# tatsy/opengl-raytracer

Hardware: AMD Instinct MI355X
Metric: Mrays/s at 1920x1080, 8 bounces (higher is better)
Workload: dtype f32

## Files before the change

opengl-raytracer_amd/csrc/glrtx.hip:

```cpp
#include "glrtx.h"

#include <hip/hip_runtime.h>

#include <algorithm>
#include <cmath>
#include <cstdarg>
#include <cstdio>
#include <cstdlib>
#include <cstring>
#include <new>
#include <limits>
#include <string>
#include <vector>

#include "glrt_host.h"
#include "pt_kernel.hip.h"
#include "lbvh.hip.h"
#include "sahl.hip.h"
#include "refit.hip.h"
#include "query.hip.h"
#include "features.hip.h"
#include "denoise.hip.h"
#include "reproject.hip.h"
#include "../host/reproject_setup.h"
// ... 1079 lines not shown
    if (fed) {
        FeedHost *fh = slot->feed_h;
        for (int i = 0; i < n_frames; i++) fh->seeds[i] = make_float2(seeds_xy[2 * i], seeds_xy[2 * i + 1]);
        __atomic_store_n(&fh->frames_pub, (unsigned)n_frames, __ATOMIC_RELEASE);
        w.feed_host = slot->feed_h_dev;
        w.feed_dev = (FeedDev *)slot->feed_d.p;
        w.feed_plane_f4 = plane_f4;
        w.feed_margin = 64 * 4 * grid;
        if (const char *v = std::getenv("GLRTX_FEED_MARGIN")) w.feed_margin = std::max(0, std::atoi(v));
    } else {
        if (n_frames > 1) {
            if ((rc = ensure(c, c->wfSeeds, (size_t)n_frames * sizeof(float2)))) return rc;
            HIP_TRY(c, hipMemcpyAsync(c->wfSeeds.p, seeds_xy, (size_t)n_frames * sizeof(float2), hipMemcpyHostToDevice, c->stream));
            w.seeds = (const float2 *)c->wfSeeds.p;
            w.seeds_in_lds = n_frames <= kLdsSeeds ? 1 : 0;
        }
        if (n_frames > 1 || slot || adapt) {
            if ((rc = ensure(c, planeBuf, (size_t)std::max(n_planes, 1) * plane_f4 * sizeof(float4)))) return rc;
            w.planes = (float4 *)planeBuf.p;
        }
    }
    w.block_paths = block_paths;
    w.gss_div = (slot && !fed) ? 0 : 4 * grid;
    if (const char *v = std::getenv("GLRTX_GSS_DIV")) w.gss_div = std::max(0, std::atoi(v));
    w.suspend_max = kSuspendMax;
    if (const char *v = std::getenv("GLRTX_SUSPEND_MAX")) w.suspend_max = std::max(0, std::min(64, std::atoi(v)));
    w.trip_limit = (int)std::min<long long>(INT32_MAX, 64ll * std::max(p->n_samples, 1) * (p->max_depth + 2) + 64);
    if (vol) w.trip_limit = (int)std::min<long long>(INT32_MAX, 64ll * std::max(p->n_samples, 1) * 9 * (p->max_depth + 2) + 64);
    if (const char *v = std::getenv("GLRTX_TRIP_LIMIT")) w.trip_limit = std::max(1, std::atoi(v));
    w.err = c->guard_dev;
    {
        const size_t max_id = ids - 1;
        const size_t max_sidx = (size_t)kWfSetPlanes * state_entries + (size_t)grid * block_paths - 1;
        const size_t slice_f4 = 2 * (size_t)2 * 2 * block_paths  + (2 * (size_t)block_paths * sizeof(unsigned) + 15) / 16 ;
        static_assert(kWgSuspendAt + (size_t)kSuspendF4 * kBlockThreads == kWgQueueF4, "the suspend area closes a workgroup's slice");
        bool ok = slice_f4 <= kWgSuspendAt && max_id < (size_t)WF_INVALID && 2 * max_sidx + 1 < (size_t)WF_INVALID && (size_t)grid * block_paths <= state_entries &&
                  (size_t)kWfStatePlanes * state_entries * sizeof(float4) < ((size_t)1 << 32) && (block_paths & (block_paths - 1)) == 0 && block_paths >= 256 &&
                  block_paths <= kWgPathsMax && slice_f4 <= kWgQueueF4 && queueBuf.bytes >= (size_t)grid * kWgQueueF4 * sizeof(float4) &&
                  stateBuf.bytes >= state_bytes && w.ids == state_entries && grid >= 1 && (size_t)grid <= wg_slots &&
                  p->max_depth <= kWfDepthMax && p->n_samples <= kWfSampleMax && workPtr != nullptr;
        if (vol) ok = ok && p->n_samples <= kWfVolSampleMax && c->ext_flags == GLRTX_EXT_VOLUME && c->have_volume && c->vol.density != nullptr &&
                      c->vol.temperature != nullptr && c->n_spheres == 0 && !vine && fetch == 0 && !compact;
        if (!fed && n_frames > 1) ok = ok && c->wfSeeds.bytes >= (size_t)n_frames * sizeof(float2);
        if (w.planes) ok = ok && planeBuf.bytes >= (size_t)std::max(n_planes, 1) * plane_f4 * sizeof(float4);
        if (adapt) ok = ok && !fed && !slot && w.planes && c->ad_selected && c->ad_tiles == (int)(total >> 6) && c->adList.bytes >= (total >> 6) * sizeof(int) &&
                      c->adMask.bytes >= (total >> 6) && c->adHalf.bytes >= (size_t)c->ad_pitch * c->owned_rows && c->ad_pitch == c->pitch_bytes;
        if (fed) ok = ok && n_frames >= 1 && n_frames <= fed_cap && fed_cap <= kFeedMaxFrames && slot->feed_d.bytes >= sizeof(FeedDev) && w.feed_host != nullptr &&
                      slot->chunks[(n_frames - 1) / kFeedChunkFrames].p != nullptr && slot->chunk_bytes == frame_bytes;
        if (!ok) return fail(c, GLRTX_EDEVICE, "internal: wgwf launch shapes inconsistent (ids %zu, max id %zu, grid %d of %zu slots (%d per CU), block_paths %d, frames %d, fed %d)", ids, max_id,
                             grid, wg_slots, per_cu, block_paths, n_frames, (int)fed);
        (void)queue_bytes_max;
    }
    glrtx_ctx::LaunchRec *rec = nullptr;
    if ((rc = next_launch_rec(c, rec))) return rc;
    if (slot && slot->used) HIP_TRY(c, hipStreamWaitEvent(rstream, slot->acc_done, 0));
    if (ctx_state && c->state_used) HIP_TRY(c, hipStreamWaitEvent(rstream, c->state_done, 0));
    HIP_TRY(c, hipMemsetAsync(workPtr, 0, sizeof(unsigned), rstream));
    if (fed) {
        hipLaunchKernelGGL(feed_prefill_kernel, dim3(1), dim3(64), 0, rstream, (FeedDev *)slot->feed_d.p, (const FeedHost *)slot->feed_h_dev, n_frames);
        HIP_TRY(c, hipGetLastError());
    }
    HIP_TRY(c, hipEventRecord(rec->ev0, rstream));
    c->last_kernel = vol ? (adapt ? "pt_render_wgwf (volume, adaptive)" : "pt_render_wgwf (volume)")
                   : adapt ? (vine ? "pt_render_wgwf (adaptive, list scan)" : "pt_render_wgwf (adaptive)") : vine ? "pt_render_wgwf (list scan)" : "pt_render_wgwf";
    c->counters_stale = c->counters_stale || c->count_rays;
    const VolArgs va = vol ? c->vol : VolArgs{};
    hipLaunchKernelGGL(kernel, dim3(grid), dim3(kBlockThreads), lds, rstream, a, w, workPtr, (float4 *)queueBuf.p, adapt ? (const int *)c->adList.p : nullptr,
// ... 2097 lines not shown
```

opengl-raytracer_amd/csrc/pt_kernel.hip.h:

```cpp
#pragma once
#include <hip/hip_runtime.h>
#include <stdint.h>

#include "trav_asm.hip.h"
#include "scan_asm.hip.h"

namespace glrtx {

constexpr int kBlockThreads = 256;
constexpr int kTile = 16;
constexpr int REF_ABSENT = INT32_MIN;
constexpr int REF_FIN = INT32_MIN;
constexpr int kMaxLdsMaterials = 256;
constexpr int kMaxLdsLights = 64;
constexpr int kTopForks = 128;

constexpr float PT_EPS = 1.0e-4f;
constexpr float PT_INFTY = 1.0e8f;
constexpr float PT_PI = 3.14159274101257324f;
constexpr float PT_2PI = 6.28318548202514648f;

struct DevScene {
    const float4 *forks;
    const float4 *nodes0;
// ... 1422 lines not shown
    int total;
    int tiles8_x;
    int refill_min;
    int block_paths;
    int gss_div;
    int suspend_max;
    int trip_limit;
    unsigned *err;
    FeedHost *feed_host;
    FeedDev *feed_dev;
    size_t feed_plane_f4;
    int feed_margin;
    const float2 *seeds;
    int seeds_in_lds;
    float4 *planes;
    int n_frames;
    int tiles_per_frame;
    DEV void split(int id, int &frame, int &pid) const {
        if (n_frames > 1) { frame = (int)((unsigned)id / (unsigned)total); pid = id - frame * total; }
        else { frame = 0; pid = id; }
    }
};
constexpr int kWfStatePlanes = 2 * kWfSetPlanes;
constexpr int kWfDepthMax = 255;
constexpr int kWfSampleMax = (1 << 20) - 1;
constexpr int kWfVolSampleMax = (1 << 16) - 1;
constexpr unsigned kWfVolShift = 24;
constexpr unsigned kWfVolPassed = 9;
constexpr unsigned WF_PENDING = 1u << 28;
constexpr unsigned WF_FINISHING = 1u << 29;
constexpr unsigned WF_RESOLVED = 1u << 30;
constexpr unsigned WF_ACCEPTED = 1u << 31;
constexpr unsigned WF_INVALID = 0xFFFFFFFFu;
constexpr int kSuspendMax = 24;
constexpr float kHitSuspended = -1.0f;
constexpr int kSuspendF4 = 4;
constexpr int kRefillMin = 16;
#ifdef GLRTX_FAULT_INJECT
constexpr unsigned kFaultPoison = 0xFFFFFFFEu;
#endif

DEV bool wf_pixel(const KernelArgs &a, const WfArgs &w, int id, int &lx, int &lrow) {
    int frame, pid;
    w.split(id, frame, pid);
    const int t = pid >> 6, k = pid & 63;
    lx = (t % w.tiles8_x) * 8 + (k & 7);
    lrow = (t / w.tiles8_x) * 8 + (k >> 3);
    return lx < a.width && lrow < a.owned_rows;
}

DEV float2 wf_seed(const KernelArgs &a, const WfArgs &w, const float *cam, int id) {
    if (w.n_frames > 1) {
        int frame, pid;
        w.split(id, frame, pid);
        if (w.seeds_in_lds) {
            const float *sd = cam + kCamFloatsPadded + 2 * frame;
            return make_float2(sd[0], sd[1]);
        }
        if (w.feed_dev != nullptr) {
            const nfloat2 v = ((glb_cf2)&w.feed_dev->seeds[0])[frame];
            return make_float2(v.x, v.y);
        }
        const nfloat2 v = ((glb_cf2)w.seeds)[frame];
        return make_float2(v.x, v.y);
    }
    return make_float2(a.seed_x, a.seed_y);
// ... 5 lines not shown
        w.split(id, frame, pid);
        typedef __attribute__((address_space(1))) nfloat4 *glb_f4;
        const glb_f4 chunk = (glb_f4)w.feed_dev->chunks[frame / kFeedChunkFrames];
        const size_t slot = (size_t)(frame % kFeedChunkFrames) * (size_t)a.n_samples + sample;
        nfloat4 v; v.x = fmin_c(Lx, 100.0f); v.y = fmin_c(Ly, 100.0f); v.z = fmin_c(Lz, 100.0f); v.w = 1.0f;
        __builtin_nontemporal_store(v, &chunk[slot * w.feed_plane_f4 + (size_t)lrow * (size_t)a.pitch_f4 + lx]);
    } else if (w.planes != nullptr) {
        int frame, pid;
        w.split(id, frame, pid);
        const size_t slot = (size_t)frame * (size_t)a.n_samples + sample;
        st_stream(&w.planes[(slot * (size_t)a.owned_rows + (size_t)lrow) * (size_t)a.pitch_f4 + lx],
                  make_float4(fmin_c(Lx, 100.0f), fmin_c(Ly, 100.0f), fmin_c(Lz, 100.0f), 1.0f));
    } else {
        float4 *px = a.accum + (size_t)lrow * a.pitch_f4 + lx;
        float4 acc = *px;
        acc.x = acc.x + fmin_c(Lx, 100.0f);
        acc.y = acc.y + fmin_c(Ly, 100.0f);
        acc.z = acc.z + fmin_c(Lz, 100.0f);
        acc.w = acc.w + 1.0f;
        *px = acc;
    }
}

DEV bool wf_start(const KernelArgs &a, const WfArgs &w, const float *cam, int id, int lx, int lrow, Rng &rng, float fcx, float fcy, Path &P, unsigned &sample) {
    for (;;) {
        if ((int)sample >= a.n_samples) return false;
        camera_ray(a, cam, rng, fcx, fcy, P);
        if (a.max_depth > 0) return true;
        wf_add_sample(a, w, id, lx, lrow, sample, 0.0f, 0.0f, 0.0f);
        sample++;
    }
}

DEV bool wf_generate_one(const KernelArgs &a, const WfArgs &w, const float *cam, int id, unsigned sidx, float4 &ray_o, float4 &ray_d) {
    int lx, lrow;
    bool go = false;
    const float2 sd = wf_seed(a, w, cam, id);
    Rng rng = {0.f, 0.f, sd.x, sd.y};
    Path P;
    unsigned sample = 0;
    if (wf_pixel(a, w, id, lx, lrow)) {
        const int gy = local_row_to_y(a, lrow);
        const float fcx = (float)lx + 0.5f, fcy = (float)gy + 0.5f;
        rng.x = fcx / (float)a.width; rng.y = fcy / (float)a.height;
        go = wf_start(a, w, cam, id, lx, lrow, rng, fcx, fcy, P, sample);
    }
    if (go) {
        st_stream(w.A(0, sidx), make_float4(P.ox, P.oy, P.oz, rng.x));
        st_stream(w.A(1, sidx), make_float4(P.dx, P.dy, P.dz, rng.y));
        st_stream(w.A(2, sidx), make_float4(1.f, 1.f, 1.f, __uint_as_float(sample << 8)));
        st_stream(w.A(3, sidx), make_float4(0.f, 0.f, 0.f, __uint_as_float((unsigned)id)));
        ray_o = make_float4(P.ox, P.oy, P.oz, __uint_as_float(sidx * 2u));
        ray_d = make_float4(P.dx, P.dy, P.dz, 0.f);
    } else st_stream(w.A(3, sidx), make_float4(0.f, 0.f, 0.f, __uint_as_float(WF_INVALID)));
    return go;
}

constexpr int kWfVolEnd = 0, kWfVolNext = 1, kWfVolExit = 2;
DEV const VolArgs *wgwf_vol();
DEV int wf_vol_trial(const KernelArgs &a, const WfArgs &w, unsigned sidx, Rng &rng, Path &P, const Hit &h, unsigned k) {
    if (h.tri < 0) { P.Lx = 1.0f; P.Ly = 0.0f; P.Lz = 1.0f; return kWfVolEnd; }
    const float ox = P.ox, oy = P.oy, oz = P.oz, dx = P.dx, dy = P.dy, dz = P.dz;
    float t = 0.0f;
    bool pass = false;
    for (int i = 0; i < 256; i++) {
        const VolArgs &vo = *wgwf_vol();
        const float dm = vo.density_max;
        t = t - lp_log(fmax_c(1.0f - pt_rand(rng), PT_EPS)) / (dm * VOL_SIGT);
        if (t >= h.t) { pass = true; break; }
        const float density = vol_lookup(vo.density, vo, ox + t * dx, oy + t * dy, oz + t * dz);
        if (density / dm > pt_rand(rng)) { pass = true; break; }
    }
    if (!pass) { P.Lx = 0.0f; P.Ly = 0.0f; P.Lz = 0.0f; return kWfVolEnd; }
    {
        unsigned si = sidx;
        asm volatile("" : "+v"(si));
        const float4 b = ld_stream(w.A(2, si)), l = ld_stream(w.A(3, si));
        P.bx = b.x; P.by = b.y; P.bz = b.z; P.Lx = l.x; P.Ly = l.y; P.Lz = l.z;
    }
    if (t >= h.t) {
        const float te = h.t + PT_EPS;
        P.ox = ox + te * dx; P.oy = oy + te * dy; P.oz = oz + te * dz;
    } else {
        P.ox = ox + t * dx; P.oy = oy + t * dy; P.oz = oz + t * dz;
        float R, G, B;
        const VolArgs &vo = *wgwf_vol();
        vol_blackbody(vol_lookup(vo.temperature, vo, P.ox, P.oy, P.oz), R, G, B);
// ... 140 lines not shown
#define GLRTX_STEPS_PER_TRIP 6
#endif
constexpr int kWgCtlWords = 32;
constexpr int kWgPathsMax = 4096;
constexpr size_t kWgSuspendAt = 8 * (size_t)kWgPathsMax + (size_t)kWgPathsMax / 2;
constexpr size_t kWgQueueF4 = kWgSuspendAt + (size_t)kSuspendF4 * kBlockThreads;
#ifndef GLRTX_PRIO_TRAVERSE
#define GLRTX_PRIO_TRAVERSE 3
#define GLRTX_PRIO_SHADE 0
#endif
#ifndef GLRTX_WGWF_WAVES
#define GLRTX_WGWF_WAVES 4
#endif

#ifdef GLRTX_PHASE_STATS
__device__ unsigned long long g_phase_cycles[8];
__device__ uint4 g_trip_log[16][64];
#define PH_STAMP(var) const unsigned long long var = __builtin_amdgcn_s_memtime()
#define PH_ADD(i, t0, t1) do { if (threadIdx.x == 0) atomicAdd(&g_phase_cycles[i], (t1) - (t0)); } while (0)
#else
#define PH_STAMP(var)
#define PH_ADD(i, t0, t1)
#endif

#ifdef GLRTX_RAY_LOG
struct RayLog { float4 *rays; uint2 *trips; unsigned long long cap_rays; unsigned cap_trips; unsigned on; };
__device__ RayLog g_ray_log;
__device__ unsigned long long g_ray_log_n;
__device__ unsigned g_ray_log_trips;
#endif

DEV int wgwf_suspend_max();

template <bool VINE, int FETCH>
DEV void wg_traverse_phase(const KernelArgs &a, const WfArgs &w, const float4 *root, int *stack, const float4 *rq, int n_rays,
                           unsigned *ray_head, unsigned *light_bits, unsigned long long &rays, float4 *suspend_area) {
    const int lane = threadIdx.x & 63;
    const uint2 *ranks = reinterpret_cast<const uint2 *>(light_bits + kWgPathsMax / 32);
    if (VINE) {
        for (;;) {
            int base = 0;
            if (lane == 0) base = (int)atomicAdd(ray_head, 64u);
            base = __builtin_amdgcn_readfirstlane(base);
            if (base >= n_rays) break;
            float4 o = make_float4(0.f, 0.f, 0.f, __uint_as_float(WF_INVALID)), d = o;
            if (base + lane < n_rays) { o = ld_stream(&rq[2 * (size_t)(base + lane)]); d = ld_stream(&rq[2 * (size_t)(base + lane) + 1]); }
            const unsigned r = __float_as_uint(o.w);
            const bool shadow = (r & 1u) != 0u;
            const Hit h = trav_scan<true>(a.sc, o.x, o.y, o.z, d.x, d.y, d.z, r != WF_INVALID, shadow ? shadow_limit(d.w, a.sc.shadow_limited) : PT_INFTY,
                                          shadow ? d.w : -__builtin_inff());
            if (r != WF_INVALID) {
                rays++;
                if (r & 1u) { if (nee_accepted(d.w, h.t, h.tri >= 0)) atomicOr(&light_bits[r >> 6], 1u << ((r >> 1) & 31u)); }
                else st_stream(w.H(r >> 1), make_float4(h.t, __int_as_float(h.tri), h.u, h.v));
            }
        }
        return;
    }
    const unsigned long long lt_mask = (1ull << lane) - 1ull;
    const float4 none = make_float4(0.f, 0.f, 0.f, __uint_as_float(WF_INVALID));
    float4 cur_o = none, cur_d = none;
    float cur_ix = 0.f, cur_iy = 0.f, cur_iz = 0.f;
    int cur_pos = 0, cur_cnt = 0;
    auto fetch = [&](float4 &o, float4 &d) -> int {
        int base = 0;
        if (lane == 0) base = (int)atomicAdd(ray_head, 64u);
        base = __builtin_amdgcn_readfirstlane(base);
        int cnt = n_rays - base;
        cnt = cnt < 0 ? 0 : (cnt > 64 ? 64 : cnt);
        if (lane < cnt) {
            o = ld_stream(&rq[2 * (size_t)(base + lane)]);
            d = ld_stream(&rq[2 * (size_t)(base + lane) + 1]);
            cur_ix = frcp(d.x); cur_iy = frcp(d.y); cur_iz = frcp(d.z);
            const bool shadow = (__float_as_uint(o.w) & 1u) != 0u;
            float t0;
            if (a.sc.root_boxed && !box_pass(root[0], root[1], o.x, o.y, o.z, cur_ix, cur_iy, cur_iz, shadow ? shadow_limit(d.w, a.sc.shadow_limited) : PT_INFTY, t0))
                d.w = __uint_as_float(__float_as_uint(d.w) | 0x80000000u);
        }
        return cnt;
    };
    cur_cnt = fetch(cur_o, cur_d);
    bool exhausted = cur_cnt == 0;
    const bool fetched_any = cur_cnt > 0;
    bool active = false;
    bool unsaved = false;
    unsigned rid = 0;
    Trav T;
    T.cur = 0; T.sp = 0;
    T.h.t = PT_INFTY; T.h.tri = -1; T.h.u = 0.f; T.h.v = 0.f;
#ifdef GLRTX_STEP_TIMING
    StepTiming step_timing;
#endif
    float4 *const susp = suspend_area + (size_t)kSuspendF4 * threadIdx.x;
    {
        const float4 s3 = susp[3];
        if (s3.z != 0.0f) {
            const float4 s0 = susp[0], s1 = susp[1], s2 = susp[2];
            susp[3] = make_float4(0.f, 0.f, 0.f, 0.f);
            T.ox = s0.x; T.oy = s0.y; T.oz = s0.z;
            rid = __float_as_uint(w.H(__float_as_uint(s0.w) >> 1)->y);
#ifdef GLRTX_FAULT_INJECT
            const bool fault_dropped = rid == kFaultPoison;
#endif
            T.dx = s1.x; T.dy = s1.y; T.dz = s1.z; T.stop_d = s1.w;
            T.ix = frcp(T.dx); T.iy = frcp(T.dy); T.iz = frcp(T.dz);
// ... 105 lines not shown
            bool fin = trav_step<true, CP>(a.sc, stack, T, ranks);
#pragma unroll
            for (int k = 1; k < GLRTX_STEPS_PER_TRIP; k++)
                if (!fin) fin = trav_step<true, CP>(a.sc, stack, T, ranks);
#else
#ifdef GLRTX_STEP_TIMING
            trav_steps_asm<FETCH>(a.sc, stack, T, (unsigned)(uintptr_t)ranks, step_timing);
#else
            trav_steps_asm<FETCH>(a.sc, stack, T, (unsigned)(uintptr_t)ranks);
#endif
            const bool fin = T.cur == REF_FIN;
#endif
            if (fin) {
                active = false;
                unsaved = true;
            }
        }
#ifdef GLRTX_PHASE_STATS
        ph_step += __builtin_amdgcn_s_memtime() - sb0;
#endif
    }
    if (unsaved) save_hit();
#ifdef GLRTX_PHASE_STATS
    if (threadIdx.x == 0) { atomicAdd(&g_phase_cycles[5], ph_refill); atomicAdd(&g_phase_cycles[6], ph_refills); atomicAdd(&g_phase_cycles[7], ph_step); }
#endif
#ifdef GLRTX_STEP_TIMING
    atomicAdd(&g_step_timing[0], (unsigned long long)step_timing.n);
    atomicAdd(&g_step_timing[1], (unsigned long long)step_timing.t);
    atomicAdd(&g_step_timing[2], (unsigned long long)step_timing.w);
#endif
}

template <bool VOL = false>
DEV void wg_shade_phase(const KernelArgs &a, const WfArgs &w, const float4 *lds_mats, const float *cam, const unsigned *light_bits, int n_paths,
                        float4 *rq_next, unsigned *n_rays_next, unsigned *n_paths_next, unsigned cur_base, unsigned next_base, unsigned long long &rays,
                        unsigned *moved) {
    const int lane = threadIdx.x & 63;
    const unsigned long long lt_mask = (1ull << lane) - 1ull;
    for (int j0 = 0; j0 < n_paths; j0 += kBlockThreads) {
        const int i = j0 + (int)threadIdx.x;
        bool push_ext = false, push_sh = false, requeue = false, has4 = false;
        unsigned id = WF_INVALID;
        float4 ro = make_float4(0.f, 0.f, 0.f, 0.f), rd = ro, rsd = ro, st2 = ro, st3 = ro, st4 = ro;
        const bool light_accepted = i < n_paths && ((light_bits[i >> 5] >> (i & 31)) & 1u) != 0u;
        if (i < n_paths)
            wf_shade_path<VOL>(a, w, lds_mats, cam, id, cur_base + (unsigned)i, light_accepted, push_ext, push_sh, requeue, ro, rd, rsd, st2, st3, st4, has4, rays);
        const unsigned long long me = __ballot(push_ext), ms = __ballot(push_sh), mq = __ballot(requeue), mp = me | ms | mq;
        const unsigned long long mv = __ballot(id != WF_INVALID);
        unsigned br = 0, bp = 0;
        if (lane == 0) {
            if (mv & ~mq) *moved = 1u;
            if (mp) {
                br = atomicAdd(n_rays_next, (unsigned)(__popcll(me) + __popcll(ms)));
                bp = atomicAdd(n_paths_next, (unsigned)__popcll(mp));
            }
        }
        br = __builtin_amdgcn_readfirstlane(br);
        bp = __builtin_amdgcn_readfirstlane(bp);
        const unsigned pos_next = bp + (unsigned)__popcll(mp & lt_mask);
        const unsigned sidx_next = next_base + pos_next;
        if (push_ext || push_sh || requeue) {
            st_stream(w.A(0, sidx_next), ro);
            st_stream(w.A(1, sidx_next), rd);
            st_stream(w.A(2, sidx_next), st2);
            st_stream(w.A(3, sidx_next), st3);
            if (has4) st_stream(w.A(4, sidx_next), st4);
        }
#ifdef GLRTX_FAULT_INJECT
        if (requeue) {
            *w.H(cur_base + (unsigned)i) = make_float4(kHitSuspended, __uint_as_float(kFaultPoison), 0.f, 0.f);
            *w.H(sidx_next) = make_float4(kHitSuspended, 0.f, 0.f, 0.f);
        }
#else
        if (requeue) *w.H(cur_base + (unsigned)i) = make_float4(kHitSuspended, __uint_as_float(sidx_next * 2u), 0.f, 0.f);
#endif
        if (push_ext) {
            float4 *r = rq_next + 2 * (size_t)(br + __popcll(me & lt_mask));
            r[0] = make_float4(ro.x, ro.y, ro.z, __uint_as_float(sidx_next * 2u));
            r[1] = make_float4(rd.x, rd.y, rd.z, 0.f);
        }
        if (push_sh) {
            float4 *r = rq_next + 2 * (size_t)(br + __popcll(me) + __popcll(ms & lt_mask));
            r[0] = make_float4(ro.x, ro.y, ro.z, __uint_as_float(pos_next * 2u + 1u));
            r[1] = rsd;
        }
    }
}

struct WgwfKernArgs {
    KernelArgs a;
    WfArgs w;
    unsigned *work_counter;
    float4 *wg_queues;
    const int *adapt_list;
    const unsigned *adapt_count;
    VolArgs vol;
};
DEV const WgwfKernArgs *wgwf_kernargs() {
    auto p = __builtin_amdgcn_kernarg_segment_ptr();
    asm volatile("" : "+s"(p));
    return (const WgwfKernArgs *)p;
}

DEV int wgwf_suspend_max() { return wgwf_kernargs()->w.suspend_max; }
DEV const VolArgs *wgwf_vol() { return &wgwf_kernargs()->vol; }

template <bool VOL = false>
DEV void wg_feed_topup(int kWgPaths, unsigned *ctl, int cur, unsigned *work_counter) {
    const WgwfKernArgs *k = wgwf_kernargs();
    FeedHost *fh = k->w.feed_host;
    FeedDev *fd = k->w.feed_dev;
    int lane = threadIdx.x;
    if constexpr (VOL) asm volatile("" : "+v"(lane));
    const int tpf = k->w.tiles_per_frame, gss_div = k->w.gss_div;
    const int np = (int)ctl[4 + cur];
// ... 90 lines not shown
                                                                                  const int * , const unsigned * , const VolArgs ) {
    constexpr bool ADAPT = (FETCH & kWgwfAdaptive) != 0;
    constexpr bool VOL = (FETCH & kWgwfVolume) != 0;
    constexpr int NODE_FETCH = FETCH & ~(kWgwfAdaptive | kWgwfVolume);
    static_assert(!VOL || (!VINE && NODE_FETCH == 0), "the V form has the one-record-per-lane fetch on DevScene::nodes only");
    extern __shared__ __attribute__((aligned(16))) unsigned char lds_raw[];
    float4 *lds_mats = reinterpret_cast<float4 *>(lds_raw);
    const int mat_f4 = a.sc.lds_head_f4;
    unsigned char *pl = lds_raw + (size_t)mat_f4 * sizeof(float4);
    int *stack = reinterpret_cast<int *>(pl) + 2 * threadIdx.x;
    pl += (size_t)2 * a.sc.stack_entries * kBlockThreads * sizeof(int);
    unsigned *ctl = reinterpret_cast<unsigned *>(pl);
    float4 *lds_root = reinterpret_cast<float4 *>(pl + kWgCtlWords * sizeof(unsigned));
    float *lds_cam = reinterpret_cast<float *>(pl + kWgCtlWords * sizeof(unsigned) + 32);
    unsigned *light_bits = reinterpret_cast<unsigned *>(pl + kWgCtlWords * sizeof(unsigned) + 32 + kCamFloatsPadded * 4 + kLdsSeeds * 8);
    if (threadIdx.x < kCamFloats) lds_cam[threadIdx.x] = a.cam[threadIdx.x];
    if (w.seeds_in_lds && (int)threadIdx.x < 2 * w.n_frames) lds_cam[kCamFloatsPadded + threadIdx.x] = reinterpret_cast<const float *>(w.seeds)[threadIdx.x];
    if (threadIdx.x == 64) lds_root[0] = a.sc.root_lo;
    if (threadIdx.x == 65) lds_root[1] = a.sc.root_hi;
    float4 *rayQ = wg_queues + (size_t)blockIdx.x * kWgQueueF4;
    if (a.sc.mats_in_lds) stage_mats(a, lds_mats);
    stage_lights(a, lds_mats);
    if (FETCH & kWgwfCompact) {
        uint2 *lds_ranks = reinterpret_cast<uint2 *>(light_bits + kWgPathsMax / 32);
        for (int i = threadIdx.x; i < a.sc.n_crank; i += kBlockThreads) lds_ranks[i] = a.sc.cranks[i];
    }

    const int kWgPaths = w.block_paths;
    unsigned long long rays = 0;
#ifdef GLRTX_PHASE_STATS
    if (threadIdx.x == 0 && (blockIdx.x & 63) == 0 && blockIdx.x / 64 < 16)
        g_trip_log[blockIdx.x / 64][0].y = (unsigned)(__builtin_amdgcn_s_memtime() >> 4);
#endif
    if (threadIdx.x == 0) { ctl[2] = 0u; ctl[3] = 0u; ctl[4] = 0u; ctl[5] = 0u; ctl[7] = 0u; ctl[10] = 0u; ctl[11] = 0u; ctl[12] = 0u; ctl[13] = 0u; ctl[14] = 0u; ctl[15] = 0u; ctl[16] = 0u; ctl[17] = 0u; ctl[18] = 0u; }
    if (!VINE) rayQ[kWgSuspendAt + (size_t)kSuspendF4 * threadIdx.x + 3] = make_float4(0.f, 0.f, 0.f, 0.f);
    int cur = 0;
    __syncthreads();
    for (;;) {
        PH_STAMP(pg0);
        unsigned tid_topup = threadIdx.x;
        asm volatile("" : "+v"(tid_topup));
        if (wgwf_kernargs()->w.feed_dev != nullptr) {
            if (tid_topup < 64u) wg_feed_topup<VOL>(kWgPaths, ctl, cur, work_counter);
        } else if (tid_topup == 0u) {
            const int n_tiles = (ADAPT ? (int)*wgwf_kernargs()->adapt_count : wgwf_kernargs()->w.tiles_per_frame) * wgwf_kernargs()->w.n_frames;
            int want = (kWgPaths - (int)ctl[4 + cur]) >> 6;
            int base = 0, got = 0;
            const int gss_div = wgwf_kernargs()->w.gss_div;
            if (want > 0 && ctl[7] == 0u && gss_div > 0) {
                const int left = n_tiles - (int)__hip_atomic_load(work_counter, __ATOMIC_RELAXED, __HIP_MEMORY_SCOPE_AGENT);
                const int share = left > 0 ? (left + gss_div - 1) / gss_div : 1;
                want = want < share ? want : share;
            }
            if (want > 0 && ctl[7] == 0u && ctl[13] == 0u) {
                base = (int)atomicAdd(work_counter, (unsigned)want);
                got = base < n_tiles ? (want < n_tiles - base ? want : n_tiles - base) : 0;
                if (base + want >= n_tiles) ctl[7] = 1u;
            }
            ctl[0] = (unsigned)base; ctl[6] = (unsigned)got; ctl[14] = 0u;
            ctl[12] = got > 0 ? 0u : ctl[12] + 1u;
        }
        __syncthreads();
        if (ctl[13] != 0u) break;
        const bool look_again = ctl[14] != 0u;
        {
            const int got = (int)ctl[6] * 64, tile0 = (int)ctl[0];
            {
                unsigned tid = threadIdx.x;
                asm volatile("" : "+v"(tid));
                if (tid < kWgPathsMax / 32) light_bits[tid] = 0u;
            }
            const int nr = (int)ctl[2 + cur], np = (int)ctl[4 + cur];
            float4 *rq_w = rayQ + 2 * ((size_t)cur * 2 * kWgPaths + nr);
            const WgwfKernArgs *kt = wgwf_kernargs();
            const unsigned new_base = kt->w.set_base(cur, (int)blockIdx.x) + (unsigned)np;
            for (int k = threadIdx.x; k < got; k += kBlockThreads) {
                int id = tile0 * 64 + k;
                if (ADAPT) {
                    const int g = tile0 + (k >> 6), n_active = (int)*kt->adapt_count;
                    const int frame = g / n_active;
                    id = frame * kt->w.total + kt->adapt_list[g - frame * n_active] * 64 + (k & 63);
                }
                float4 ro = make_float4(0.f, 0.f, 0.f, __uint_as_float(WF_INVALID)), rd = ro;
                const bool go = wf_generate_one(kt->a, kt->w, lds_cam, id, new_base + (unsigned)k, ro, rd);
                rq_w[2 * k] = ro;
                rq_w[2 * k + 1] = rd;
                (void)go;
            }
            __syncthreads();
            if (tid_topup == 0u) { ctl[2 + cur] = (unsigned)(nr + got); ctl[4 + cur] = (unsigned)(np + got); ctl[1] = 0u; }
        }
        __syncthreads();
        PH_STAMP(pg1);
        PH_ADD(0, pg0, pg1);
        const int n_rays = (int)ctl[2 + cur], n_paths = (int)ctl[4 + cur];
        if (n_paths == 0) {
            if (look_again) continue;
            break;
        }
        const float4 *rq = rayQ + 2 * ((size_t)cur * 2 * kWgPaths);

#ifdef GLRTX_RAY_LOG
        if (g_ray_log.on) {
            if (threadIdx.x == 0) {
                const unsigned long long base = atomicAdd(&g_ray_log_n, (unsigned long long)n_rays);
                ctl[9] = 0u;
                if (base + (unsigned long long)n_rays <= g_ray_log.cap_rays) {
                    const unsigned t = atomicAdd(&g_ray_log_trips, 1u);
                    if (t < g_ray_log.cap_trips) { g_ray_log.trips[t] = make_uint2((unsigned)base, (unsigned)n_rays); ctl[8] = (unsigned)base; ctl[9] = 1u; }
                }
            }
            __syncthreads();
            if (ctl[9]) {
                float4 *dst = g_ray_log.rays + 2 * (size_t)ctl[8];
                for (int i = threadIdx.x; i < 2 * n_rays; i += kBlockThreads) dst[i] = rq[i];
            }
            __syncthreads();
        }
#endif
        PH_STAMP(pt0);
        __builtin_amdgcn_s_setprio(GLRTX_PRIO_TRAVERSE);
        wg_traverse_phase<VINE, NODE_FETCH>(a, w, lds_root, stack, rq, n_rays, &ctl[1], light_bits, rays, rayQ + kWgSuspendAt);
        __builtin_amdgcn_s_setprio(GLRTX_PRIO_SHADE);
        PH_STAMP(pt1);
        __syncthreads();
        PH_STAMP(pt2);
        PH_ADD(1, pt0, pt1);
        PH_ADD(2, pt1, pt2);

        const WgwfKernArgs *ks = wgwf_kernargs();
        wg_shade_phase<VOL>(ks->a, ks->w, lds_mats, lds_cam, light_bits, n_paths, rayQ + 2 * ((size_t)(cur ^ 1) * 2 * kWgPaths),
                            &ctl[2 + (cur ^ 1)], &ctl[4 + (cur ^ 1)], ks->w.set_base(cur, (int)blockIdx.x), ks->w.set_base(cur ^ 1, (int)blockIdx.x), rays, &ctl[10]);
        PH_STAMP(ps1);
        __syncthreads();
        PH_STAMP(ps2);
        PH_ADD(3, pt2, ps1);
        PH_ADD(4, ps1, ps2);
#ifdef GLRTX_PHASE_STATS
        if (threadIdx.x == 0 && (blockIdx.x & 63) == 0 && blockIdx.x / 64 < 16) {
            uint4 *lg = g_trip_log[blockIdx.x / 64];
            const unsigned n = lg[0].x + 1u;
            if (n < 64u) { lg[n] = make_uint4((unsigned)n_rays, (unsigned)n_paths, (unsigned)(pt2 - pt0), (unsigned)(ps2 - pt2)); lg[0].x = n; }
        }
#endif
        unsigned tid_end = threadIdx.x;
        asm volatile("" : "+v"(tid_end));
        if (tid_end == 0u) {
            ctl[2 + cur] = 0u; ctl[4 + cur] = 0u;
            const bool idle = n_rays == 0 && ctl[10] == 0u;
            ctl[10] = 0u;
            const unsigned idle_trips = idle ? ctl[11] + 1u : 0u;
            ctl[11] = idle_trips;
            const WgwfKernArgs *kg = wgwf_kernargs();
            const unsigned code = idle_trips >= 2u ? 1u : (ctl[12] > (unsigned)kg->w.trip_limit ? 2u : 0u);
            if (code != 0u) {
                unsigned *e = kg->w.err;
                unsigned wg;
                asm volatile("v_mov_b32 %0, %1" : "=v"(wg) : "s"((unsigned)blockIdx.x));
                __hip_atomic_store(e + 1, wg, __ATOMIC_RELAXED, __HIP_MEMORY_SCOPE_SYSTEM);
                __hip_atomic_store(e + 2, ctl[12], __ATOMIC_RELAXED, __HIP_MEMORY_SCOPE_SYSTEM);
                __hip_atomic_store(e + 3, ctl[4 + (cur ^ 1)], __ATOMIC_RELAXED, __HIP_MEMORY_SCOPE_SYSTEM);
                __hip_atomic_store(e, code, __ATOMIC_RELEASE, __HIP_MEMORY_SCOPE_SYSTEM);
                ctl[13] = 1u;
            }
        }
        cur ^= 1;
    }
#ifdef GLRTX_PHASE_STATS
    if (threadIdx.x == 0 && (blockIdx.x & 63) == 0 && blockIdx.x / 64 < 16)
        g_trip_log[blockIdx.x / 64][0].z = (unsigned)(__builtin_amdgcn_s_memtime() >> 4);
#endif
    flush_rays<COUNT_RAYS>(a, rays);
}

#ifdef GLRTX_RAY_LOG
template <int FETCH>
__global__ __launch_bounds__(kBlockThreads, GLRTX_WGWF_WAVES) void pt_replay_traverse(const KernelArgs a, const WfArgs w, unsigned *work_counter, float4 *wg_queues,
                                                                                      const float4 *log, const uint2 *trips, int n_trips) {
    extern __shared__ __attribute__((aligned(16))) unsigned char lds_raw[];
    const int mat_f4 = a.sc.lds_head_f4;
    unsigned char *pl = lds_raw + (size_t)mat_f4 * sizeof(float4);
    int *stack = reinterpret_cast<int *>(pl) + 2 * threadIdx.x;
    pl += (size_t)2 * a.sc.stack_entries * kBlockThreads * sizeof(int);
    unsigned *ctl = reinterpret_cast<unsigned *>(pl);
    float4 *lds_root = reinterpret_cast<float4 *>(pl + kWgCtlWords * sizeof(unsigned));
    unsigned *light_bits = reinterpret_cast<unsigned *>(pl + kWgCtlWords * sizeof(unsigned) + 32 + kCamFloatsPadded * 4 + kLdsSeeds * 8);
    if (threadIdx.x == 64) lds_root[0] = a.sc.root_lo;
    if (threadIdx.x == 65) lds_root[1] = a.sc.root_hi;
    float4 *rayQ = wg_queues + (size_t)blockIdx.x * kWgQueueF4;
    rayQ[kWgSuspendAt + (size_t)kSuspendF4 * threadIdx.x + 3] = make_float4(0.f, 0.f, 0.f, 0.f);
    unsigned long long rays = 0;
    __syncthreads();
    for (;;) {
        if (threadIdx.x == 0) { ctl[0] = atomicAdd(work_counter, 1u); ctl[1] = 0u; }
        if (threadIdx.x < kWgPathsMax / 32) light_bits[threadIdx.x] = 0u;
        __syncthreads();
        const unsigned t = ctl[0];
        if (t >= (unsigned)n_trips) break;
        const uint2 tr = trips[t];
        __builtin_amdgcn_s_setprio(GLRTX_PRIO_TRAVERSE);
        wg_traverse_phase<false, FETCH>(a, w, lds_root, stack, log + 2 * (size_t)tr.x, (int)tr.y, &ctl[1], light_bits, rays, rayQ + kWgSuspendAt);
        __builtin_amdgcn_s_setprio(GLRTX_PRIO_SHADE);
        __syncthreads();
    }
    flush_rays<true>(a, rays);
}
#endif

__global__ __launch_bounds__(256) void accumulate_planes_kernel(float4 *accum, int pitch_f4, int width, int rows, const float4 *planes,
                                                                int n_planes) {
    const int x = blockIdx.x * 64 + (threadIdx.x & 63);
    const int y = blockIdx.y * 4 + (threadIdx.x >> 6);
    if (x >= width || y >= rows) return;
    const size_t at = (size_t)y * pitch_f4 + x, plane = (size_t)rows * pitch_f4;
    float4 acc = accum[at];
    for (int k = 0; k < n_planes; k++) {
        const float4 v = planes[(size_t)k * plane + at];
        acc.x = acc.x + v.x; acc.y = acc.y + v.y; acc.z = acc.z + v.z;
        acc.w = acc.w + 1.0f;
    }
    accum[at] = acc;
}

__global__ __launch_bounds__(64) void feed_prefill_kernel(FeedDev *fd, const FeedHost *fh, int n_frames) {
    const int lane = threadIdx.x;
    for (int f = lane; f < n_frames; f += 64) fd->seeds[f] = (unsigned long long)__float_as_uint(fh->seeds[f].x) | ((unsigned long long)__float_as_uint(fh->seeds[f].y) << 32);
    for (int c = lane; c <= (n_frames - 1) / kFeedChunkFrames; c += 64) fd->chunks[c] = (unsigned long long)fh->chunks[c];
    if (lane == 0) fd->frames_known = (unsigned)n_frames;
}

__global__ __launch_bounds__(256) void accumulate_feed_kernel(float4 *accum, int pitch_f4, int width, int rows, const FeedDev *fd, int n_samples) {
    const int x = blockIdx.x * 64 + (threadIdx.x & 63);
    const int y = blockIdx.y * 4 + (threadIdx.x >> 6);
    if (x >= width || y >= rows) return;
// ... 232 lines not shown
```

Measured before the change: 10320.

## Read extension rays straight from path state instead of a duplicated ray queue

Extension rays are no longer copied into the per-workgroup ray queue. Traversal now fetches them directly from path-state planes 0 and 1, which are compacted at the front of the path set, while requeued and shadow-only paths are packed from the back. Only shadow rays still go through the queue, which halves its slice size and removes one redundant write and read per extension ray. The cost is more complex index arithmetic and three atomic counters per wave, plus a no-ray sentinel that must be written for invalid generated paths.

Result: no change. 10260 (-0.6%).

```diff
diff --git a/opengl-raytracer_amd/csrc/glrtx.hip b/opengl-raytracer_amd/csrc/glrtx.hip
--- a/opengl-raytracer_amd/csrc/glrtx.hip
+++ b/opengl-raytracer_amd/csrc/glrtx.hip
@@ -1135,7 +1135,7 @@
     {
         const size_t max_id = ids - 1;
         const size_t max_sidx = (size_t)kWfSetPlanes * state_entries + (size_t)grid * block_paths - 1;
-        const size_t slice_f4 = 2 * (size_t)2 * 2 * block_paths  + (2 * (size_t)block_paths * sizeof(unsigned) + 15) / 16 ;
+        const size_t slice_f4 = 2 * (size_t)2 * block_paths;
         static_assert(kWgSuspendAt + (size_t)kSuspendF4 * kBlockThreads == kWgQueueF4, "the suspend area closes a workgroup's slice");
         bool ok = slice_f4 <= kWgSuspendAt && max_id < (size_t)WF_INVALID && 2 * max_sidx + 1 < (size_t)WF_INVALID && (size_t)grid * block_paths <= state_entries &&
                   (size_t)kWfStatePlanes * state_entries * sizeof(float4) < ((size_t)1 << 32) && (block_paths & (block_paths - 1)) == 0 && block_paths >= 256 &&
diff --git a/opengl-raytracer_amd/csrc/pt_kernel.hip.h b/opengl-raytracer_amd/csrc/pt_kernel.hip.h
--- a/opengl-raytracer_amd/csrc/pt_kernel.hip.h
+++ b/opengl-raytracer_amd/csrc/pt_kernel.hip.h
@@ -1478,6 +1478,7 @@
 constexpr unsigned WF_RESOLVED = 1u << 30;
 constexpr unsigned WF_ACCEPTED = 1u << 31;
 constexpr unsigned WF_INVALID = 0xFFFFFFFFu;
+constexpr unsigned kWfNoRay = 0xFFFFFFFFu;
 constexpr int kSuspendMax = 24;
 constexpr float kHitSuspended = -1.0f;
 constexpr int kSuspendF4 = 4;
@@ -1549,7 +1550,7 @@
     }
 }
 
-DEV bool wf_generate_one(const KernelArgs &a, const WfArgs &w, const float *cam, int id, unsigned sidx, float4 &ray_o, float4 &ray_d) {
+DEV bool wf_generate_one(const KernelArgs &a, const WfArgs &w, const float *cam, int id, unsigned sidx) {
     int lx, lrow;
     bool go = false;
     const float2 sd = wf_seed(a, w, cam, id);
@@ -1567,9 +1568,12 @@
         st_stream(w.A(1, sidx), make_float4(P.dx, P.dy, P.dz, rng.y));
         st_stream(w.A(2, sidx), make_float4(1.f, 1.f, 1.f, __uint_as_float(sample << 8)));
         st_stream(w.A(3, sidx), make_float4(0.f, 0.f, 0.f, __uint_as_float((unsigned)id)));
-        ray_o = make_float4(P.ox, P.oy, P.oz, __uint_as_float(sidx * 2u));
-        ray_d = make_float4(P.dx, P.dy, P.dz, 0.f);
-    } else st_stream(w.A(3, sidx), make_float4(0.f, 0.f, 0.f, __uint_as_float(WF_INVALID)));
+    } else {
+        const float4 no_ray = make_float4(__uint_as_float(kWfNoRay), 0.f, 0.f, 0.f);
+        st_stream(w.A(0, sidx), no_ray);
+        st_stream(w.A(1, sidx), no_ray);
+        st_stream(w.A(3, sidx), make_float4(0.f, 0.f, 0.f, __uint_as_float(WF_INVALID)));
+    }
     return go;
 }
 
@@ -1776,8 +1780,33 @@
 
 DEV int wgwf_suspend_max();
 
+DEV int wf_fetch_chunk(const WfArgs &w, const float4 *rq, int n_front, int n_sh, unsigned cur_base, int base, int lane, float4 &o, float4 &d) {
+    const int front_end = (n_front + 63) & ~63;
+    int cnt;
+    o = make_float4(0.f, 0.f, 0.f, __uint_as_float(WF_INVALID));
+    d = o;
+    if (base < front_end) {
+        const int have = n_front - base;
+        cnt = base + 64 < front_end + n_sh ? 64 : have;
+        if (lane < have) {
+            const unsigned sidx = cur_base + (unsigned)(base + lane);
+            o = ld_stream(w.A(0, sidx));
+            d = ld_stream(w.A(1, sidx));
+            const bool no_ray = (__float_as_uint(o.x) & __float_as_uint(d.x)) == kWfNoRay;
+            o.w = __uint_as_float(no_ray ? WF_INVALID : sidx * 2u);
+            d.w = 0.f;
+        }
+    } else {
+        const int at = base - front_end;
+        cnt = n_sh - at;
+        cnt = cnt < 0 ? 0 : (cnt > 64 ? 64 : cnt);
+        if (lane < cnt) { o = ld_stream(&rq[2 * (size_t)(at + lane)]); d = ld_stream(&rq[2 * (size_t)(at + lane) + 1]); }
+    }
+    return cnt;
+}
+
 template <bool VINE, int FETCH>
-DEV void wg_traverse_phase(const KernelArgs &a, const WfArgs &w, const float4 *root, int *stack, const float4 *rq, int n_rays,
+DEV void wg_traverse_phase(const KernelArgs &a, const WfArgs &w, const float4 *root, int *stack, const float4 *rq, int n_front, int n_sh, unsigned cur_base,
                            unsigned *ray_head, unsigned *light_bits, unsigned long long &rays, float4 *suspend_area) {
     const int lane = threadIdx.x & 63;
     const uint2 *ranks = reinterpret_cast<const uint2 *>(light_bits + kWgPathsMax / 32);
@@ -1786,9 +1815,8 @@
             int base = 0;
             if (lane == 0) base = (int)atomicAdd(ray_head, 64u);
             base = __builtin_amdgcn_readfirstlane(base);
-            if (base >= n_rays) break;
-            float4 o = make_float4(0.f, 0.f, 0.f, __uint_as_float(WF_INVALID)), d = o;
-            if (base + lane < n_rays) { o = ld_stream(&rq[2 * (size_t)(base + lane)]); d = ld_stream(&rq[2 * (size_t)(base + lane) + 1]); }
+            float4 o, d;
+            if (wf_fetch_chunk(w, rq, n_front, n_sh, cur_base, base, lane, o, d) == 0) break;
             const unsigned r = __float_as_uint(o.w);
             const bool shadow = (r & 1u) != 0u;
             const Hit h = trav_scan<true>(a.sc, o.x, o.y, o.z, d.x, d.y, d.z, r != WF_INVALID, shadow ? shadow_limit(d.w, a.sc.shadow_limited) : PT_INFTY,
@@ -1810,11 +1838,8 @@
         int base = 0;
         if (lane == 0) base = (int)atomicAdd(ray_head, 64u);
         base = __builtin_amdgcn_readfirstlane(base);
-        int cnt = n_rays - base;
-        cnt = cnt < 0 ? 0 : (cnt > 64 ? 64 : cnt);
+        const int cnt = wf_fetch_chunk(w, rq, n_front, n_sh, cur_base, base, lane, o, d);
         if (lane < cnt) {
-            o = ld_stream(&rq[2 * (size_t)(base + lane)]);
-            d = ld_stream(&rq[2 * (size_t)(base + lane) + 1]);
             cur_ix = frcp(d.x); cur_iy = frcp(d.y); cur_iz = frcp(d.z);
             const bool shadow = (__float_as_uint(o.w) & 1u) != 0u;
             float t0;
@@ -1986,32 +2011,34 @@
 }
 
 template <bool VOL = false>
-DEV void wg_shade_phase(const KernelArgs &a, const WfArgs &w, const float4 *lds_mats, const float *cam, const unsigned *light_bits, int n_paths,
-                        float4 *rq_next, unsigned *n_rays_next, unsigned *n_paths_next, unsigned cur_base, unsigned next_base, unsigned long long &rays,
-                        unsigned *moved) {
+DEV void wg_shade_phase(const KernelArgs &a, const WfArgs &w, const float4 *lds_mats, const float *cam, const unsigned *light_bits, int n_front, int n_paths,
+                        float4 *rq_next, unsigned *next, unsigned cur_base, unsigned next_base, unsigned long long &rays, unsigned *moved) {
     const int lane = threadIdx.x & 63;
     const unsigned long long lt_mask = (1ull << lane) - 1ull;
     for (int j0 = 0; j0 < n_paths; j0 += kBlockThreads) {
-        const int i = j0 + (int)threadIdx.x;
+        const int j = j0 + (int)threadIdx.x;
+        const int i = j < n_front ? j : j + (w.block_paths - n_paths);
         bool push_ext = false, push_sh = false, requeue = false, has4 = false;
         unsigned id = WF_INVALID;
         float4 ro = make_float4(0.f, 0.f, 0.f, 0.f), rd = ro, rsd = ro, st2 = ro, st3 = ro, st4 = ro;
-        const bool light_accepted = i < n_paths && ((light_bits[i >> 5] >> (i & 31)) & 1u) != 0u;
-        if (i < n_paths)
+        const bool light_accepted = j < n_paths && ((light_bits[i >> 5] >> (i & 31)) & 1u) != 0u;
+        if (j < n_paths)
             wf_shade_path<VOL>(a, w, lds_mats, cam, id, cur_base + (unsigned)i, light_accepted, push_ext, push_sh, requeue, ro, rd, rsd, st2, st3, st4, has4, rays);
-        const unsigned long long me = __ballot(push_ext), ms = __ballot(push_sh), mq = __ballot(requeue), mp = me | ms | mq;
+        const unsigned long long me = __ballot(push_ext), ms = __ballot(push_sh), mq = __ballot(requeue), mb = (ms | mq) & ~me;
         const unsigned long long mv = __ballot(id != WF_INVALID);
-        unsigned br = 0, bp = 0;
+        unsigned bf = 0, bb = 0, bs = 0;
         if (lane == 0) {
             if (mv & ~mq) *moved = 1u;
-            if (mp) {
-                br = atomicAdd(n_rays_next, (unsigned)(__popcll(me) + __popcll(ms)));
-                bp = atomicAdd(n_paths_next, (unsigned)__popcll(mp));
-            }
-        }
-        br = __builtin_amdgcn_readfirstlane(br);
-        bp = __builtin_amdgcn_readfirstlane(bp);
-        const unsigned pos_next = bp + (unsigned)__popcll(mp & lt_mask);
+            if (me | mb) {
+                bf = atomicAdd(&next[0], (unsigned)__popcll(me));
+                bb = atomicAdd(&next[1], (unsigned)__popcll(mb));
+                bs = atomicAdd(&next[2], (unsigned)__popcll(ms));
+            }
+        }
+        bf = __builtin_amdgcn_readfirstlane(bf);
+        bb = __builtin_amdgcn_readfirstlane(bb);
+        bs = __builtin_amdgcn_readfirstlane(bs);
+        const unsigned pos_next = push_ext ? bf + (unsigned)__popcll(me & lt_mask) : (unsigned)w.block_paths - 1u - (bb + (unsigned)__popcll(mb & lt_mask));
         const unsigned sidx_next = next_base + pos_next;
         if (push_ext || push_sh || requeue) {
             st_stream(w.A(0, sidx_next), ro);
@@ -2028,13 +2055,8 @@
 #else
         if (requeue) *w.H(cur_base + (unsigned)i) = make_float4(kHitSuspended, __uint_as_float(sidx_next * 2u), 0.f, 0.f);
 #endif
-        if (push_ext) {
-            float4 *r = rq_next + 2 * (size_t)(br + __popcll(me & lt_mask));
-            r[0] = make_float4(ro.x, ro.y, ro.z, __uint_as_float(sidx_next * 2u));
-            r[1] = make_float4(rd.x, rd.y, rd.z, 0.f);
-        }
         if (push_sh) {
-            float4 *r = rq_next + 2 * (size_t)(br + __popcll(me) + __popcll(ms & lt_mask));
+            float4 *r = rq_next + 2 * (size_t)(bs + __popcll(ms & lt_mask));
             r[0] = make_float4(ro.x, ro.y, ro.z, __uint_as_float(pos_next * 2u + 1u));
             r[1] = rsd;
         }
@@ -2191,7 +2213,7 @@
     if (threadIdx.x == 0 && (blockIdx.x & 63) == 0 && blockIdx.x / 64 < 16)
         g_trip_log[blockIdx.x / 64][0].y = (unsigned)(__builtin_amdgcn_s_memtime() >> 4);
 #endif
-    if (threadIdx.x == 0) { ctl[2] = 0u; ctl[3] = 0u; ctl[4] = 0u; ctl[5] = 0u; ctl[7] = 0u; ctl[10] = 0u; ctl[11] = 0u; ctl[12] = 0u; ctl[13] = 0u; ctl[14] = 0u; ctl[15] = 0u; ctl[16] = 0u; ctl[17] = 0u; ctl[18] = 0u; }
+    if (threadIdx.x == 0) { ctl[24] = 0u; ctl[25] = 0u; ctl[26] = 0u; ctl[28] = 0u; ctl[29] = 0u; ctl[30] = 0u; ctl[4] = 0u; ctl[5] = 0u; ctl[7] = 0u; ctl[10] = 0u; ctl[11] = 0u; ctl[12] = 0u; ctl[13] = 0u; ctl[14] = 0u; ctl[15] = 0u; ctl[16] = 0u; ctl[17] = 0u; ctl[18] = 0u; }
     if (!VINE) rayQ[kWgSuspendAt + (size_t)kSuspendF4 * threadIdx.x + 3] = make_float4(0.f, 0.f, 0.f, 0.f);
     int cur = 0;
     __syncthreads();
@@ -2229,10 +2251,9 @@
                 asm volatile("" : "+v"(tid));
                 if (tid < kWgPathsMax / 32) light_bits[tid] = 0u;
             }
-            const int nr = (int)ctl[2 + cur], np = (int)ctl[4 + cur];
-            float4 *rq_w = rayQ + 2 * ((size_t)cur * 2 * kWgPaths + nr);
+            const int nf = (int)ctl[24 + 4 * cur], np = (int)ctl[4 + cur];
             const WgwfKernArgs *kt = wgwf_kernargs();
-            const unsigned new_base = kt->w.set_base(cur, (int)blockIdx.x) + (unsigned)np;
+            const unsigned new_base = kt->w.set_base(cur, (int)blockIdx.x) + (unsigned)nf;
             for (int k = threadIdx.x; k < got; k += kBlockThreads) {
                 int id = tile0 * 64 + k;
                 if (ADAPT) {
@@ -2240,46 +2261,50 @@
                     const int frame = g / n_active;
                     id = frame * kt->w.total + kt->adapt_list[g - frame * n_active] * 64 + (k & 63);
                 }
-                float4 ro = make_float4(0.f, 0.f, 0.f, __uint_as_float(WF_INVALID)), rd = ro;
-                const bool go = wf_generate_one(kt->a, kt->w, lds_cam, id, new_base + (unsigned)k, ro, rd);
-                rq_w[2 * k] = ro;
-                rq_w[2 * k + 1] = rd;
-                (void)go;
+                (void)wf_generate_one(kt->a, kt->w, lds_cam, id, new_base + (unsigned)k);
             }
             __syncthreads();
-            if (tid_topup == 0u) { ctl[2 + cur] = (unsigned)(nr + got); ctl[4 + cur] = (unsigned)(np + got); ctl[1] = 0u; }
+            if (tid_topup == 0u) { ctl[24 + 4 * cur] = (unsigned)(nf + got); ctl[4 + cur] = (unsigned)(np + got); ctl[1] = 0u; }
         }
         __syncthreads();
         PH_STAMP(pg1);
         PH_ADD(0, pg0, pg1);
-        const int n_rays = (int)ctl[2 + cur], n_paths = (int)ctl[4 + cur];
+        const int n_front = (int)ctl[24 + 4 * cur], n_paths = (int)ctl[4 + cur], n_sh = (int)ctl[26 + 4 * cur];
+        const int n_rays = n_front + n_sh;
         if (n_paths == 0) {
             if (look_again) continue;
             break;
         }
-        const float4 *rq = rayQ + 2 * ((size_t)cur * 2 * kWgPaths);
+        const float4 *rq = rayQ + 2 * ((size_t)cur * kWgPaths);
 
 #ifdef GLRTX_RAY_LOG
         if (g_ray_log.on) {
+            const int n_log = ((n_front + 63) & ~63) + n_sh;
             if (threadIdx.x == 0) {
-                const unsigned long long base = atomicAdd(&g_ray_log_n, (unsigned long long)n_rays);
+                const unsigned long long base = atomicAdd(&g_ray_log_n, (unsigned long long)n_log);
                 ctl[9] = 0u;
-                if (base + (unsigned long long)n_rays <= g_ray_log.cap_rays) {
+                if (base + (unsigned long long)n_log <= g_ray_log.cap_rays) {
                     const unsigned t = atomicAdd(&g_ray_log_trips, 1u);
-                    if (t < g_ray_log.cap_trips) { g_ray_log.trips[t] = make_uint2((unsigned)base, (unsigned)n_rays); ctl[8] = (unsigned)base; ctl[9] = 1u; }
+                    if (t < g_ray_log.cap_trips) { g_ray_log.trips[t] = make_uint2((unsigned)base, (unsigned)n_log); ctl[8] = (unsigned)base; ctl[9] = 1u; }
                 }
             }
             __syncthreads();
             if (ctl[9]) {
                 float4 *dst = g_ray_log.rays + 2 * (size_t)ctl[8];
-                for (int i = threadIdx.x; i < 2 * n_rays; i += kBlockThreads) dst[i] = rq[i];
+                const unsigned log_base = wgwf_kernargs()->w.set_base(cur, (int)blockIdx.x);
+                for (int b = 64 * (int)(threadIdx.x >> 6); b < n_log; b += kBlockThreads) {
+                    float4 o, d;
+                    const int lane = (int)(threadIdx.x & 63u);
+                    if (lane < wf_fetch_chunk(w, rq, n_front, n_sh, log_base, b, lane, o, d)) { dst[2 * (b + lane)] = o; dst[2 * (b + lane) + 1] = d; }
+                }
             }
             __syncthreads();
         }
 #endif
         PH_STAMP(pt0);
         __builtin_amdgcn_s_setprio(GLRTX_PRIO_TRAVERSE);
-        wg_traverse_phase<VINE, NODE_FETCH>(a, w, lds_root, stack, rq, n_rays, &ctl[1], light_bits, rays, rayQ + kWgSuspendAt);
+        wg_traverse_phase<VINE, NODE_FETCH>(a, w, lds_root, stack, rq, n_front, n_sh, wgwf_kernargs()->w.set_base(cur, (int)blockIdx.x), &ctl[1], light_bits, rays,
+                                            rayQ + kWgSuspendAt);
         __builtin_amdgcn_s_setprio(GLRTX_PRIO_SHADE);
         PH_STAMP(pt1);
         __syncthreads();
@@ -2288,8 +2313,8 @@
         PH_ADD(2, pt1, pt2);
 
         const WgwfKernArgs *ks = wgwf_kernargs();
-        wg_shade_phase<VOL>(ks->a, ks->w, lds_mats, lds_cam, light_bits, n_paths, rayQ + 2 * ((size_t)(cur ^ 1) * 2 * kWgPaths),
-                            &ctl[2 + (cur ^ 1)], &ctl[4 + (cur ^ 1)], ks->w.set_base(cur, (int)blockIdx.x), ks->w.set_base(cur ^ 1, (int)blockIdx.x), rays, &ctl[10]);
+        wg_shade_phase<VOL>(ks->a, ks->w, lds_mats, lds_cam, light_bits, n_front, n_paths, rayQ + 2 * ((size_t)(cur ^ 1) * kWgPaths),
+                            &ctl[24 + 4 * (cur ^ 1)], ks->w.set_base(cur, (int)blockIdx.x), ks->w.set_base(cur ^ 1, (int)blockIdx.x), rays, &ctl[10]);
         PH_STAMP(ps1);
         __syncthreads();
         PH_STAMP(ps2);
@@ -2305,7 +2330,8 @@
         unsigned tid_end = threadIdx.x;
         asm volatile("" : "+v"(tid_end));
         if (tid_end == 0u) {
-            ctl[2 + cur] = 0u; ctl[4 + cur] = 0u;
+            ctl[24 + 4 * cur] = 0u; ctl[25 + 4 * cur] = 0u; ctl[26 + 4 * cur] = 0u; ctl[4 + cur] = 0u;
+            ctl[4 + (cur ^ 1)] = ctl[24 + 4 * (cur ^ 1)] + ctl[25 + 4 * (cur ^ 1)];
             const bool idle = n_rays == 0 && ctl[10] == 0u;
             ctl[10] = 0u;
             const unsigned idle_trips = idle ? ctl[11] + 1u : 0u;
@@ -2358,7 +2384,7 @@
         if (t >= (unsigned)n_trips) break;
         const uint2 tr = trips[t];
         __builtin_amdgcn_s_setprio(GLRTX_PRIO_TRAVERSE);
-        wg_traverse_phase<false, FETCH>(a, w, lds_root, stack, log + 2 * (size_t)tr.x, (int)tr.y, &ctl[1], light_bits, rays, rayQ + kWgSuspendAt);
+        wg_traverse_phase<false, FETCH>(a, w, lds_root, stack, log + 2 * (size_t)tr.x, 0, (int)tr.y, 0u, &ctl[1], light_bits, rays, rayQ + kWgSuspendAt);
         __builtin_amdgcn_s_setprio(GLRTX_PRIO_SHADE);
         __syncthreads();
     }
```
